# TUD-UCB-Boda/boda-1

Hardware: AMD Instinct MI355X
Metric: per-op GFLOPS and % fp32 roofline on sgemm-ops-full + conv-ops (AlexNet/NiN/GoogLeNet) (higher is better)
Workload: dtype f32; 1 GPU; sgemm-ops-full.txt + conv-ops-1-5-20-nin-alex-gn.txt + op_sigs_full.txt (one main-kernel launch per op per step); launch=hipGraph replay of each step, ops=399, units=399, ops_cut_into_panels=0, parallelism=op-shard1 (LPT, no collective), plat=hip:MI355X:gfx950:sramecc+:xnack-

## Files before the change

boda-1_amd/csrc/bh_common.h:

```cpp
#pragma once
#include <hip/hip_runtime.h>
#include <hip/hip_ext.h>
#include <stdint.h>
#include <algorithm>
#include <dlfcn.h>
#include <map>
#include <mutex>
#include <string>
#include <vector>
#include "boda_hip.h"
#include "bh_lanes.h"

namespace bh {
struct op_scope;
}
struct bh_lane {
  hipStream_t stream = nullptr;
  void *ws = nullptr;
  size_t ws_bytes = 0;
  void *cnt = nullptr;
  uint64_t cnt_n = 0;
  bool forked = false;
};
struct bh_sched {
  int lanes = 1;
  double narrow_us = 0;
  bool capturing = false;
  bh_lane lane[bh_lanes::MAX_LANES];
  std::vector<hipEvent_t> ev;
  size_t ev_used = 0;
  bh_lanes::tracker trk;
  size_t hw_ws = 0;
  bh::op_scope *scope = nullptr;
  uint32_t used_mask = 0;
  uint32_t cur[4] = {0, 0, 0, 0};
  uint32_t stats[4] = {0, 0, 0, 0};
  std::vector<uint32_t> cur_trace, trace;
};

struct bh_ctx {
  int device = 0;
  hipStream_t stream = nullptr;
  hipDeviceProp_t prop{};
  std::vector<hipEvent_t> events;
  int events_used = 0;
  int ovr_cfg[2] = {-1, -1};
  uint32_t ovr_splits[2] = {0, 0};
  int ovr_red[2] = {0, 0};
  int ovr_wt[2] = {-1, -1};
  std::vector<hipGraphExec_t> graphs;
  void *stamps = nullptr;
  hipEvent_t t_start = nullptr;
  hipEvent_t t_stop = nullptr;
  double stamp_hz = 100e6;
  void *wpack = nullptr;
  size_t wpack_bytes = 0;
  int bck_cfg[2] = {-1, -1};
  int bck_splits[2] = {0, 0};
  void *bckw = nullptr;
  size_t bckw_bytes = 0;
  std::vector<void *> retired;
  bh_sched sched;
};

namespace bh {

int fail(int code, const std::string &msg);
int ok();

int check_launch(const char *what);

int launch(bh_ctx *ctx, const void *kernel, dim3 grid, dim3 block, void **args, bool first, bool last,
           const char *what, uint32_t shmem = 0);

struct op_scope {
  bh_ctx *c;
  bh_lanes::access acc;
  double est_us = 0;
  bool narrow = false;
  bool resolved = false;
  bool pin0 = false;
  int lane = 0;
// ... 159 lines not shown
```

boda-1_amd/csrc/bh_direct.hip:

```cpp
#include "bh_gemm_dev.h"

namespace bhk {
static int launch_dc(bh_ctx *ctx, const cfg_t &c, const bh::conv_call &cc, GemmArgs &p, const route_t &r);
namespace {

template <int KX, int WPM>
constexpr int dc_koff(int tap, int KK) {
  return tap < KK ? (tap / KX) * WPM + tap % KX : 0;
}

template <int KX, int S, int WPM>
constexpr int dc_koffp(int tap, int KK) {
  return tap < KK ? (tap / KX) * WPM + ((tap % KX) % S) * (WPM / S) + (tap % KX) / S : 0;
}
template <int KY, int KX, int S, int WPM>
struct dc_pkinds {
  static constexpr int KK = KY * KX, KK2 = (KK + 1) / 2;
  struct tab_t {
    int nk;
    int dk[32];
    int kind[KK2];
  };
  static constexpr tab_t make() {
    tab_t t{};
// ... 22 lines not shown
}

template <int KY, int KX, int S, int WPM, int RIN, int TM, int TN, int D, int V4 = 0, int PSL = 0, int PFO = 0>
__global__ __launch_bounds__(256) void dc_kernel(GemmArgs p) {
  constexpr int NW = 4;
  constexpr int NPX = NW * 32 * TN, OCT = 32 * TM;
  constexpr int KK = KY * KX, KK2 = (KK + 1) / 2;
  constexpr int WPC = 2 * KK2 * OCT / 4;
  constexpr int LWA = (WPC + NW * 64 - 1) / (NW * 64);
  constexpr int WREG = LWA * NW * 256;
  constexpr int SF = RIN * WPM;
  constexpr int PW = V4 ? 4 : 1;
  static_assert(WPM % PW == 0, "16-B strip rows");
  static_assert(!PSL || (!V4 && WPM % S == 0), "phase-split strip: dword DMA, whole phases per row");
  constexpr int WS = WPM / S;
  constexpr int LWB = (SF / PW + NW * 64 - 1) / (NW * 64);
  constexpr int SREG = LWB * NW * 64 * PW;
  constexpr int BREG = NW * 64;
  constexpr int SLOT = WREG + SREG + BREG;
  constexpr int LW = LWA + LWB + 1;
  static_assert(D >= 2 && (D - 2) * LW <= 63, "vmcnt range");
  static_assert(OCT % 4 == 0 && OCT <= BREG, "16-B weight pieces, biases of one tile");
  constexpr int PF = PFO > 0 ? PFO : (TM * TN >= 4 ? 1 : (TM * TN >= 2 ? 2 : 3));
  constexpr int IS = (KK2 + 1) / 2 > 1 ? (KK2 + 1) / 2 : 1;
  constexpr int NST = TM * TN * 4;
  constexpr int ISS = KK2 > 2 * NST ? 2 * NST : KK2;
  __shared__ __attribute__((aligned(16))) float smem[D * SLOT];

  const int tid = threadIdx.x, lane = tid & 63;
  const int wave = __builtin_amdgcn_readfirstlane(tid >> 6);
  const int kh = lane >> 5, li = lane & 31;
  KT(0);

  const uint32_t G = gridDim.x, b0 = blockIdx.x;
  const uint32_t ntile = p.total_it;
  const uint32_t my_tiles = b0 < ntile ? (ntile - b0 + G - 1) / G : 0;
  auto decode = [&](uint32_t t, uint32_t &oc0, uint32_t &img, uint32_t &p0) {
    const uint32_t rest = fdiv(t, p.ipt_m, p.ipt_s);
    oc0 = (t - rest * p.ipt) * OCT;
    img = fdiv(rest, p.tm_m, p.tm_s);
    p0 = (rest - img * p.tiles_n) * NPX;
  };

  const __amdgpu_buffer_rsrc_t rsw = make_rsrc(p.a, p.a_bytes);
  const __amdgpu_buffer_rsrc_t rsi = make_rsrc(p.b, p.b_bytes);
  const __amdgpu_buffer_rsrc_t rsbias = make_rsrc(p.bias, p.bias ? p.M * 4u : 0u);
  uint32_t wrel[LWA], wc4[LWA], srel[LWB], srow[LWB];
#pragma unroll
  for (int j = 0; j < LWA; ++j) {
    const uint32_t e = (uint32_t)((wave * LWA + j) * 64 + lane);
    const uint32_t tap = e / (OCT / 4);
    wc4[j] = tap < (uint32_t)KK ? 4 * (e % (OCT / 4)) : 0xffffu;
    wrel[j] = (tap * p.IC * p.lda + 4 * (e % (OCT / 4))) * 4u;
  }
  const uint32_t pxa = V4 ? (p.px ? 4u : 0u) : p.px;
#pragma unroll
  for (int j = 0; j < LWB; ++j) {
    const uint32_t e = (uint32_t)((wave * LWB + j) * 64 + lane) * PW;
    const uint32_t r = e / WPM, q = e - (e / WPM) * WPM;
    const uint32_t c = PSL ? (q % WS) * S + q / WS : q;
    const int x = (int)c - (int)pxa;
    srow[j] = ((r < (uint32_t)RIN) & ((uint32_t)x < p.W)) ? r : 0xffffu;
    srel[j] = (r * p.W + (uint32_t)x) * 4u;
  }

  uint32_t tvo[LW];
  auto plan_tile = [&](uint32_t i) {
// ... 233 lines not shown
#endif
}

template <int KY, int KX, int S, int WPM, int RIN, int TM, int NW, int D, int V4, int ICMAX, int DBG = 0, int PFO = 0,
          int PSL = 0>
__global__ __launch_bounds__(NW * 64) void dcr_kernel(GemmArgs p) {
  constexpr int NT = NW * 64, NPX = NW * 32, OCT = 32 * TM;
  constexpr int KK = KY * KX, KK2 = (KK + 1) / 2;
  constexpr int WPC = 2 * KK2 * OCT / 4;
  constexpr int LWA = (WPC + NT - 1) / NT;
  constexpr int WREGC = LWA * NT * 4;
  constexpr int BREG = ((OCT + 63) / 64) * 64;
  constexpr int SF = RIN * WPM;
  constexpr int PW = V4 ? 4 : 1;
  static_assert(WPM % PW == 0, "16-B strip rows");
  static_assert(!PSL || (!V4 && WPM % S == 0), "phase-split strip: dword DMA, whole phases per row");
  constexpr int WS = WPM / S;
  constexpr int LWB = (SF / PW + NT - 1) / NT;
  constexpr int SREG = LWB * NT * PW;
  static_assert(D >= 2 && (D - 2) * LWB <= 63, "vmcnt range");
  static_assert(OCT % 4 == 0 && BREG <= NT, "16-B weight pieces, one bias DMA per wave at most");
  constexpr int PF = PFO > 0 ? PFO : (TM >= 2 ? 2 : 3);
  constexpr int IS = (KK2 + 1) / 2 > 1 ? (KK2 + 1) / 2 : 1;
  constexpr int NST = TM * 4;
  constexpr int ISS = KK2 > 2 * NST ? 2 * NST : KK2;
  __shared__ __attribute__((aligned(16))) float smem[ICMAX * WREGC + BREG + D * SREG];
  float *const wres = smem, *const bres = smem + ICMAX * WREGC, *const ring = bres + BREG;

  const int tid = threadIdx.x, lane = tid & 63;
  const int wave = __builtin_amdgcn_readfirstlane(tid >> 6);
  const int kh = lane >> 5, li = lane & 31;
  KT(0);

  const uint32_t G = gridDim.x, b0 = blockIdx.x;
  const uint32_t ntile = p.total_it;
  const uint32_t my_tiles = b0 < ntile ? (ntile - b0 + G - 1) / G : 0;
  const uint32_t oc0 = (b0 - fdiv(b0, p.ipt_m, p.ipt_s) * p.ipt) * OCT;
  auto decode = [&](uint32_t t, uint32_t &img, uint32_t &p0) {
    const uint32_t rest = fdiv(t, p.ipt_m, p.ipt_s);
    img = fdiv(rest, p.tm_m, p.tm_s);
    p0 = (rest - img * p.tiles_n) * NPX;
  };
  const __amdgpu_buffer_rsrc_t rsw = make_rsrc(p.a, p.a_bytes);
  const __amdgpu_buffer_rsrc_t rsi = make_rsrc(p.b, p.b_bytes);
  const __amdgpu_buffer_rsrc_t rsbias = make_rsrc(p.bias, p.bias ? p.M * 4u : 0u);

#pragma unroll
  for (int j = 0; j < LWA; ++j) {
    const uint32_t e = (uint32_t)((j * NW + wave) * 64 + lane), tap = e / (OCT / 4), c4 = 4 * (e % (OCT / 4));
    const uint32_t off = oob_unless((tap < (uint32_t)KK) & (oc0 + c4 < p.lda), (tap * p.IC * p.lda + oc0 + c4) * 4u);
    for (uint32_t ic = 0; ic < p.IC; ++ic) dma16s(rsw, wres + ic * WREGC + (j * NW + wave) * 256, off, ic * p.lda * 4u);
  }
  if (64 * wave < BREG)
    dma4(rsbias, bres + 64 * wave, oob_unless(oc0 + 64 * wave + lane < p.M, (oc0 + 64 * wave + lane) * 4u));

  const uint32_t pxa = V4 ? (p.px ? 4u : 0u) : p.px;
  uint32_t srel[LWB], srow[LWB], tvo[LWB];
#pragma unroll
  for (int j = 0; j < LWB; ++j) {
    const uint32_t e = (uint32_t)((wave * LWB + j) * 64 + lane) * PW;
    const uint32_t r = e / WPM, q = e - r * WPM;
    const uint32_t c = PSL ? (q % WS) * S + q / WS : q;
    const int x = (int)c - (int)pxa;
    srow[j] = ((r < (uint32_t)RIN) & ((uint32_t)x < p.W)) ? r : 0xffffu;
    srel[j] = (r * p.W + (uint32_t)x) * 4u;
  }
  auto plan_tile = [&](uint32_t i) {
// ... 302 lines not shown
  const uint32_t KY = cc.KY, KX = cc.KX, sy = cc.sy, sx = cc.sx;
  if ((int)KY != c.ky || (int)KX != c.kx || (int)sy != c.stride || (int)sx != c.stride)
    return bh::fail(BH_UNSUP, std::string("conv: direct config ") + c.name + " is for another kernel / stride");
  const bool v4 = c.v4 != 0;
  if (v4 && (p.W % 4 || p.px > 4))
    return bh::fail(BH_UNSUP, std::string("conv: 16-B strip pieces need W % 4 == 0, pad <= 4 for ") + c.name);
  const uint32_t pxa = v4 ? (p.px ? 4u : 0u) : p.px;
  const uint64_t maxcol = (uint64_t)pxa + (uint64_t)(p.OW - 1) * sx + KX - 1 - p.px;
  if (pxa + p.W > (uint32_t)c.wpm || maxcol >= (uint64_t)c.wpm)
    return bh::fail(BH_UNSUP, std::string("conv: input row too wide for ") + c.name);
  const uint32_t npx = (uint32_t)c.BN, OW = p.OW, OHW = p.OHW;
  const uint32_t tiles = (OHW + npx - 1) / npx;
  for (uint32_t t = 0; t < tiles; ++t) {
    const uint32_t a = t * npx, b = std::min(OHW, a + npx) - 1;
    if ((b / OW - a / OW) * sy + KY > (uint32_t)c.strip_rows)
      return bh::fail(BH_UNSUP, std::string("conv: pixel tile spans too many input rows for ") + c.name);
  }
  const uint64_t out_bytes = (uint64_t)cc.B * p.OCOHW * 4;
  if (out_bytes >= 0x7fffff00ull) return bh::fail(BH_UNSUP, "conv: output too large for the direct kernel");
  p.c_bytes = (uint32_t)out_bytes;
  const uint32_t octiles = (p.M + c.BM - 1) / c.BM;
  const uint64_t ntile = (uint64_t)cc.B * tiles * octiles;
  if (ntile >= (1u << 31)) return bh::fail(BH_UNSUP, "conv: too many tiles");
  if (c.icmax && p.IC > (uint32_t)c.icmax)
    return bh::fail(BH_UNSUP, std::string("conv: ") + c.name + " keeps at most " + std::to_string(c.icmax) +
                                  " input channels' weights resident");
  const void *k = (const void *)c.k[A_KVEC][B_DIRECT][0];
  const int bpc = bh::occupancy(k, c.NT);
  uint32_t G = (uint32_t)std::min<uint64_t>(ntile, (uint64_t)bh::num_cus(ctx) * std::min(bpc, 4));
  if (c.icmax) G = std::max(octiles, G / octiles * octiles);
  p.total_it = (uint32_t)ntile;
  p.tiles_n = tiles;
  p.ipt = octiles;
  bh::set_fd(tiles, p.tm_m, p.tm_s);
  bh::set_fd(octiles, p.ipt_m, p.ipt_s);
  bh::set_fd(OW, p.ow_m, p.ow_s);
  bh::set_trace(ctx, p);
  void *args[] = {&p};
  return bh::launch(ctx, k, dim3(G, 1, 1), dim3(c.NT), args, r.first, true, "conv_direct");
}

}
```

boda-1_amd/csrc/bh_gemm.hip:

```cpp
#include "bh_common.h"
#include "bh_gemm_dev.h"

namespace {

using namespace bhk;


template <int BM, int BN, int BK, int TM, int TN, int WAVES_M, int WAVES_N, int ALD, int BLD, int SPL>
__global__ __launch_bounds__(WAVES_M *WAVES_N * 64) void gemm_kernel(GemmArgs p) {
  constexpr int NT = WAVES_M * WAVES_N * 64;
  constexpr int WM = TM * 32, WN = TN * 32;
  static_assert(BM == WM * WAVES_M && BN == WN * WAVES_N, "tile shape");
  static_assert(BK % 8 == 0, "BK must be a multiple of 8");
  constexpr bool IM = (BLD == B_IM2COL || BLD == B_IM1X1);
  constexpr bool AMM = (ALD == A_MVEC || ALD == A_MSCALAR);
  static_assert(!IM || (NT % BN == 0), "im2col loader needs NT % BN == 0");
  constexpr int A_LDS = AMM ? BM * (BK + APAD) : BK * BM;
  constexpr int B_LDS = BK * BN;
  constexpr int AST = BK + APAD;

  __shared__ __attribute__((aligned(16))) float smem[2 * (A_LDS + B_LDS) + (IM ? BM : 0)];
  float *const As = smem;
  float *const Bs = smem + 2 * A_LDS;
  float *const Lbias = smem + 2 * (A_LDS + B_LDS);
// ... 798 lines not shown
uint32_t resolve_splits(cfg_t const &c, choice_t const &ch, uint32_t M, uint32_t N, uint32_t K, uint32_t ncu) {
  uint32_t tiles = ((M + c.BM - 1) / c.BM) * ((N + c.BN - 1) / c.BN);
  uint32_t nkt = (K + c.BK - 1) / c.BK;
  uint32_t S = ch.splits ? ch.splits : plan_splits(tiles, K, c.BK, ncu);
  S = std::max(1u, std::min(S, nkt));
  uint32_t ks = ((nkt + S - 1) / S) * c.BK;
  return (K + ks - 1) / ks;
}

int launch_gemm(bh_ctx *ctx, int op, choice_t const &ch, int ald, int bld, GemmArgs &p, const char *what,
                bool first = true) {
  cfg_t const &c = cfgs(op)[ch.cfg];
  p.tiles_m = (p.M + c.BM - 1) / c.BM;
  p.tiles_n = (p.N + c.BN - 1) / c.BN;
  bh::set_trace(ctx, p);
  const uint64_t nblk = (uint64_t)p.tiles_m * p.tiles_n;
  if (nblk > 0x7fffffffu) return bh::fail(BH_UNSUP, std::string(what) + ": grid too large");
  const uint32_t ncu = bh::num_cus(ctx);
  bh::scratch_t sc;
  p.tbm = c.BM;
  p.tbn = c.BN;
  if (bld == B_IMTAB && !c.k[ald][bld][0]) bld = B_IM2COL;
  if (bld == B_IMTAP && !c.k[ald][bld][0]) bld = B_IMT2;
  if (bld == B_IM1X1S && !c.k[ald][bld][0]) bld = B_IM1X1;
  if (is_gv(c)) {
    kern_t k = c.k[ald][bld][0];
    if (!k) return bh::fail(BH_ERR, std::string(what) + ": gv loader not instantiated");
    const uint32_t gran = (uint32_t)c.BK;
    const uint32_t ktg = (p.K + gran - 1) / gran;
    uint32_t S = ch.splits ? ch.splits : (uint32_t)std::max<uint64_t>(1, (1024 + nblk - 1) / nblk);
    S = std::max(1u, std::min(S, ktg));
    p.ks = ((ktg + S - 1) / S) * gran;
    S = (p.K + p.ks - 1) / p.ks;
    void *args[] = {&p};
    if (S > 1) {
      if (int rc = bh::scratch(ctx, (size_t)S * nblk * c.BM * c.BN * 4, nblk, sc)) return rc;
      p.ws = sc.ws;
      p.cnt = sc.cnt;
    }
    return bh::launch(ctx, (const void *)k, dim3((uint32_t)nblk, S, 1), dim3(c.NT), args, first, true, what);
  }
  if (c.family == F_STREAMK) {
    kern_t k = c.k[ald][bld][0];
    if (!k) return bh::fail(BH_ERR, std::string(what) + ": loader combination not instantiated");
    const uint32_t ipt = (p.K + c.BK - 1) / c.BK;
    if (nblk * ipt >= (1ull << 31)) return bh::fail(BH_UNSUP, std::string(what) + ": too many K iterations");
    const uint32_t dflt_bpc = (uint32_t)std::max(1, std::min(2, 163840 / c.lds_bytes));
    const bh::sk_grid g = bh::plan_sk_grid(nblk, ipt, ncu, ch.splits, dflt_bpc, 4);
    p.ipt = ipt;
    p.ipb = g.ipb;
    p.total_it = (uint32_t)g.total;
    set_fd(ipt, p.ipt_m, p.ipt_s);
    set_fd(p.tiles_m, p.tm_m, p.tm_s);
    if (int rc = bh::scratch(ctx, (size_t)2 * g.G * c.BM * c.BN * 4, nblk, sc)) return rc;
    p.ws = sc.ws;
    p.cnt = sc.cnt;
    void *args[] = {&p};
    return bh::launch(ctx, (const void *)k, dim3((uint32_t)g.G, 1, 1), dim3(c.NT), args, first, true, what);
  }
  const uint32_t S = resolve_splits(c, ch, p.M, p.N, p.K, ncu);
  const uint32_t nkt = (p.K + c.BK - 1) / c.BK;
  p.ks = ((nkt + S - 1) / S) * c.BK;
  int red = S <= 1 ? 0 : (ch.red ? ch.red : (nblk >= 64 || S > 4 ? 1 : 2));
  if (red == 2 && (uint64_t)S * nblk * c.BM * c.BN * 4 >= 0x7fffff00ull) red = 1;
  if (bld == B_IM1X1V && !c.k[ald][bld][red]) bld = B_IM1X1;
  kern_t k = c.k[ald][bld][red];
// ... 282 lines not shown
```

boda-1_amd/csrc/bh_gemm_dev.h:

```cpp
#pragma once
#include "bh_common.h"
#include "bh_skgrid.h"

namespace bhk {

typedef float f32x16 __attribute__((ext_vector_type(16)));
typedef float f32x4v __attribute__((ext_vector_type(4)));
typedef float f32x2v __attribute__((ext_vector_type(2)));

enum { A_KVEC = 0, A_KSCALAR = 1, A_MVEC = 2, A_MSCALAR = 3 };
enum { B_KVEC = 0, B_KSCALAR = 1, B_IM2COL = 2, B_IM1X1 = 3, B_IM1X1V = 4, B_IMT2 = 5, B_FC = 6, B_IMTAB = 7,
       B_IMTAP = 8, B_IM1X1S = 9, B_DIRECT = 10, NBLD = 11 };
constexpr int TAB_MAX = 512;

constexpr uint32_t OOB = 0x80000000u;
constexpr int APAD = 4;

struct GemmArgs {
  const float *a, *b;
  float *c;
  const float *bias;
  float *ws;
  uint32_t *cnt;
  uint32_t M, N, K;
  uint32_t lda, ldb, ldc;
  uint32_t tbm, tbn;
  uint32_t ks;
  uint32_t a_bytes, b_bytes;
  uint32_t c_bytes;
  uint32_t tiles_m, tiles_n;
  int relu;
  int cvec;
  int wt;
  const float *res;
  uint32_t H, W, KX, KYX, sy, sx, py, px, OW, OHW, HW, ICHW, OCOHW;
  uint32_t kyx_m, kyx_s, kx_m, kx_s, ohw_m, ohw_s, ow_m, ow_s;
  uint32_t IC, ic_m, ic_s;
  uint32_t ipt, ipb, total_it, ipt_m, ipt_s, tm_m, tm_s;
#ifdef BH_KTRACE
  unsigned long long *trace;
#endif
};

#ifdef BH_KTRACE
#define KT(k)                                                                                     \
  do {                                                                                            \
    if (threadIdx.x == 0)                                                                         \
      p.trace[((size_t)blockIdx.y * gridDim.x + blockIdx.x) * 8 + (k)] = wall_clock64();          \
  } while (0)
#else
#define KT(k) \
  do {        \
  } while (0)
#endif

__device__ __forceinline__ uint32_t fdiv(uint32_t n, uint32_t m, uint32_t s) {
  return (__umulhi(n, m) + n) >> s;
}

__device__ __forceinline__ __amdgpu_buffer_rsrc_t make_rsrc(const void *p, uint32_t bytes) {
  return __builtin_amdgcn_make_buffer_rsrc(const_cast<void *>(p), (short)0, (int)bytes, 0x00020000);
}
__device__ __forceinline__ uint32_t oob_unless(bool ok, uint32_t off) { return ok ? off : OOB; }
__device__ __forceinline__ f32x4v ld4(__amdgpu_buffer_rsrc_t r, uint32_t off) {
  return __builtin_bit_cast(f32x4v, __builtin_amdgcn_raw_buffer_load_b128(r, off, 0, 0));
}
__device__ __forceinline__ float ld1(__amdgpu_buffer_rsrc_t r, uint32_t off) {
  return __builtin_bit_cast(float, __builtin_amdgcn_raw_buffer_load_b32(r, off, 0, 0));
}

__device__ __forceinline__ uint32_t xcd_contig(uint32_t bid, uint32_t G) {
  const uint32_t xcd = bid & 7, q = G >> 3, r = G & 7;
  return (xcd < r ? xcd * (q + 1) : r * (q + 1) + (xcd - r) * q) + (bid >> 3);
}

__device__ __forceinline__ void map_tile(uint32_t bid, uint32_t tiles_m, uint32_t tiles_n, uint32_t &tm,
                                         uint32_t &tn) {
  uint32_t wgid = xcd_contig(bid, tiles_m * tiles_n);
  const uint32_t G = 8;
  uint32_t per_group = G * tiles_n;
  uint32_t group = wgid / per_group;
  uint32_t first_m = group * G;
  uint32_t gsm = min(tiles_m - first_m, G);
  uint32_t rem = wgid - group * per_group;
  tm = first_m + rem % gsm;
  tn = rem / gsm;
}

template <int N>
struct fvec;
template <>
struct fvec<1> { typedef float t; };
template <>
struct fvec<2> { typedef f32x2v t; };
template <>
struct fvec<4> { typedef f32x4v t; };

template <int N>
__device__ __forceinline__ float vget(const typename fvec<N>::t &v, int i) {
  if constexpr (N == 1) return v;
  else return v[i];
}

constexpr int AUX_SC1 = 16;
#ifndef BH_AUX_OUT
#define BH_AUX_OUT 0
#endif
// ... 277 lines not shown
```

boda-1_amd/csrc/bh_gv.hip:

```cpp
#include "bh_gemm_dev.h"

namespace bhk {
namespace {

typedef float f32x4t __attribute__((ext_vector_type(4)));


template <int R, int C, int NW>
struct gv_geom {
  static constexpr int NT = NW * 64, BMr = 16 * R, NC = 16 * C;
  static constexpr int TSZ = BMr * NC;
  static constexpr int NCH = TSZ / 4, CH = (NCH + NT - 1) / NT;
  static_assert(NCH % NT == 0 || NT % NCH == 0, "float4 chunks per thread");
};

template <int R, int C, int NW>
__device__ __forceinline__ void gv_bias(const GemmArgs &p, uint32_t m0, int tid, float (&bias_r)[gv_geom<R, C, NW>::CH]) {
  using G = gv_geom<R, C, NW>;
  const bool has = G::NCH % G::NT == 0 || tid < G::NCH;
#pragma unroll
  for (int j = 0; j < G::CH; ++j) {
    const uint32_t m = m0 + 4 * (uint32_t)(tid + j * G::NT) / G::NC;
    bias_r[j] = (has && p.bias && m < p.M) ? p.bias[m] : 0.0f;
  }
}

template <int R, int C, int NW, int RS, int CX = 1>
__device__ __forceinline__ void gv_finish(const GemmArgs &p, f32x4t (&acc)[R][C], float *red, uint32_t tm, uint32_t tn,
                                          int tid, int wave, int lane,
                                          const float (&bias_r)[gv_geom<R, C, NW>::CH]) {
  using G = gv_geom<R, C, NW>;
  constexpr int NT = G::NT, NC = G::NC, TSZ = G::TSZ, NCH = G::NCH, CH = G::CH;
  uint32_t *const flag = (uint32_t *)(red + NW * TSZ);
  const int i = lane & 15, g = lane >> 4;
  const uint32_t tile = blockIdx.x, split = blockIdx.y;
  {
    float *const Rw = red + wave * TSZ;
#pragma unroll
    for (int r = 0; r < R; ++r)
#pragma unroll
      for (int c = 0; c < C; ++c)
#pragma unroll
        for (int j = 0; j < 4; ++j) {
          const int row = RS == 1 ? 16 * r + 4 * g + j : RS * (4 * g + j) + r;
          Rw[row * NC + (CX > 1 ? CX * i + c : 16 * c + i)] = acc[r][c][j];
        }
  }
  __syncthreads();
  const bool has = NCH % NT == 0 || tid < NCH;
  f32x4v v[CH];
#pragma unroll
  for (int j = 0; j < CH; ++j) {
    const int ch = has ? tid + j * NT : 0;
    v[j] = *(const f32x4v *)&red[4 * ch];
#pragma unroll
    for (int w = 1; w < NW; ++w) v[j] += *(const f32x4v *)&red[w * TSZ + 4 * ch];
  }
  constexpr int IMODE = 1;
  if (gridDim.y == 1) {
    if (has) {
#pragma unroll
      for (int j = 0; j < CH; ++j) finish_store_b<IMODE, NC>(p, tm, tn, (uint32_t)(tid + j * NT), v[j], bias_r[j]);
    }
#ifdef BH_KTRACE
    asm volatile("s_waitcnt vmcnt(0)" ::: "memory");
    KT(4);
#endif
    return;
// ... 22 lines not shown
  f32x4v sum[CH];
#pragma unroll
  for (int j = 0; j < CH; ++j) sum[j] = f32x4v{0.0f, 0.0f, 0.0f, 0.0f};
  const uint32_t S = gridDim.y;
  for (uint32_t q = 0; q < S; q += 4) {
    f32x4v x[4][CH];
#pragma unroll
    for (int i2 = 0; i2 < 4; ++i2)
#pragma unroll
      for (int j = 0; j < CH; ++j)
        x[i2][j] = __builtin_bit_cast(
            f32x4v, __builtin_amdgcn_raw_buffer_load_b128(
                        rall, oob_unless(q + i2 < S, (q + i2) * tstep + (tile * TSZ + 4 * (uint32_t)(tid + j * NT)) * 4), 0,
                        AUX_SC1));
#pragma unroll
    for (int i2 = 0; i2 < 4; ++i2)
#pragma unroll
      for (int j = 0; j < CH; ++j)
        if (q + i2 < S) sum[j] += x[i2][j];
  }
#pragma unroll
  for (int j = 0; j < CH; ++j) finish_store_b<IMODE, NC>(p, tm, tn, (uint32_t)(tid + j * NT), sum[j], bias_r[j]);
}

template <int R, int C, int NW, int NG, int DB, int BLD>
__global__ __launch_bounds__(NW * 64) void gv_kernel(GemmArgs p) {
  using G = gv_geom<R, C, NW>;
  constexpr int BMr = G::BMr, NC = G::NC, KB = 16 * NG;
  __shared__ __attribute__((aligned(16))) float red[NW * G::TSZ + 4];

  const int tid = threadIdx.x, lane = tid & 63;
  const int wave = __builtin_amdgcn_readfirstlane(tid >> 6);
  KT(0);
  const uint32_t tm = blockIdx.x % p.tiles_m, tn = blockIdx.x / p.tiles_m, split = blockIdx.y;
  const uint32_t m0 = tm * BMr;
  const uint32_t kq = p.ks / NW;
  const uint32_t kw0 = split * p.ks + wave * kq;
  const uint32_t kw1 = min(p.K, kw0 + kq);
  const int i = lane & 15, g = lane >> 4;

  const __amdgpu_buffer_rsrc_t rsa = make_rsrc(p.a, p.a_bytes);
  const __amdgpu_buffer_rsrc_t rsb = make_rsrc(p.b, p.b_bytes);
  uint32_t arow[R];
#pragma unroll
  for (int r = 0; r < R; ++r) {
    const uint32_t m = m0 + 16 * r + i;
    arow[r] = oob_unless(m < p.M, m * p.lda * 4u);
  }
  uint32_t bcol[C];
  int iy0[C], ix0[C];
#pragma unroll
  for (int c = 0; c < C; ++c) {
    const uint32_t n = tn * NC + 16 * c + i;
    iy0[c] = 0;
    ix0[c] = 0;
    if constexpr (BLD == B_FC) {
      bcol[c] = oob_unless(n < p.N, n * p.K * 4u);
    } else {
      const uint32_t img = fdiv(n, p.ohw_m, p.ohw_s), pix = n - img * p.OHW;
      if constexpr (BLD == B_IM1X1) {
        bcol[c] = oob_unless(n < p.N, (img * p.ICHW + pix) * 4u);
      } else {
        const uint32_t oy = fdiv(pix, p.ow_m, p.ow_s), ox = pix - oy * p.OW;
        iy0[c] = (int)(oy * p.sy) - (int)p.py;
        ix0[c] = (int)(ox * p.sx) - (int)p.px;
        bcol[c] = (uint32_t)((int)(img * p.ICHW) + iy0[c] * (int)p.W + ix0[c]);
        if (n >= p.N) iy0[c] = -(1 << 29);
// ... 45 lines not shown
#pragma unroll
    for (int gg = 0; gg < NG; ++gg)
#pragma unroll
      for (int q = 0; q < 4; ++q)
#pragma unroll
        for (int r = 0; r < R; ++r)
#pragma unroll
          for (int c = 0; c < C; ++c)
            acc[r][c] = __builtin_amdgcn_mfma_f32_16x16x4f32(a[gg][r][q], b[gg][c][q], acc[r][c], 0, 0, 0);
  };
  uint32_t kb = kw0;
  if constexpr (DB) {
    if (kb < kw1) load_batch(kb, a0, b0);
    while (kb < kw1) {
      const uint32_t k1 = kb + KB;
      if (k1 < kw1) load_batch(k1, a1, b1);
      mma_batch(a0, b0);
      if (kb == kw0) KT(1);
      if (k1 >= kw1) break;
      const uint32_t k2 = k1 + KB;
      if (k2 < kw1) load_batch(k2, a0, b0);
      mma_batch(a1, b1);
      kb = k2;
    }
  } else {
    for (; kb < kw1; kb += KB) {
      load_batch(kb, a0, b0);
      mma_batch(a0, b0);
      if (kb == kw0) KT(1);
    }
  }

  KT(2);
  gv_finish<R, C, NW, 1>(p, acc, red, tm, tn, tid, wave, lane, bias_r);
}

template <int R>
__device__ __forceinline__ typename fvec<R>::t ldv(__amdgpu_buffer_rsrc_t r, uint32_t voff, uint32_t soff) {
  if constexpr (R == 4)
    return __builtin_bit_cast(f32x4v, __builtin_amdgcn_raw_buffer_load_b128(r, voff, soff, 0));
  else if constexpr (R == 2)
    return __builtin_bit_cast(f32x2v, __builtin_amdgcn_raw_buffer_load_b64(r, voff, soff, 0));
  else
    return __builtin_bit_cast(float, __builtin_amdgcn_raw_buffer_load_b32(r, voff, soff, 0));
}

template <int R, int C, int NW, int NG, int DB, int BLD, int PD = 0, int CX = 1>
__global__ __launch_bounds__(NW * 64) void gvp_kernel(GemmArgs p) {
  static_assert(BLD == B_IMTAP || BLD == B_IM1X1S || BLD == B_IM1X1 || BLD == B_FC,
                "gvp loaders: one-tap im2col, 1x1 or ipconv");
  constexpr bool AO = BLD == B_IM1X1 || BLD == B_FC;
  static_assert(CX == 1 || (CX == C && (CX == 2 || CX == 4) && BLD != B_IMTAP), "column interleave: 1x1, CX == C");
  using G = gv_geom<R, C, NW>;
  constexpr int BMr = G::BMr, NC = G::NC, KB = 16 * NG;
  typedef typename fvec<R>::t av_t;
  __shared__ __attribute__((aligned(16))) float red[NW * G::TSZ + 4];

  const int tid = threadIdx.x, lane = tid & 63;
  const int wave = __builtin_amdgcn_readfirstlane(tid >> 6);
  KT(0);
  const uint32_t tm = blockIdx.x % p.tiles_m, tn = blockIdx.x / p.tiles_m, split = blockIdx.y;
  const uint32_t m0 = tm * BMr;
  const uint32_t kq = p.ks / NW;
  const uint32_t kw0 = split * p.ks + wave * kq;
  const uint32_t kw1 = min(p.K, kw0 + kq);
  const int i = lane & 15, g = lane >> 4;
  const __amdgpu_buffer_rsrc_t rsa = make_rsrc(p.a, p.a_bytes);
  const __amdgpu_buffer_rsrc_t rsb = make_rsrc(p.b, p.b_bytes);
  const uint32_t lda4 = p.lda * 4u, hw4 = p.HW * 4u;
  const uint32_t arow = oob_unless(m0 + R * i < p.lda, (m0 + R * i) * 4u + g * lda4);
  uint32_t arow_o[AO ? R : 1];
#pragma unroll
  for (int r = 0; r < (AO ? R : 1); ++r) {
    const uint32_t m = m0 + 16 * r + i;
    arow_o[r] = oob_unless(m < p.M, (m * p.lda + 4 * g) * 4u);
  }
  uint32_t bcol[C];
  int iy0[C], ix0[C];
#pragma unroll
  for (int c = 0; c < C; ++c) {
    const uint32_t n = CX > 1 ? tn * NC + CX * i : tn * NC + 16 * c + i;
    const uint32_t img = fdiv(n, p.ohw_m, p.ohw_s), pix = n - img * p.OHW;
    iy0[c] = 0;
    ix0[c] = 0;
    if constexpr (BLD == B_FC) {
      bcol[c] = oob_unless(n < p.N, (n * p.ICHW + 4 * g) * 4u);
    } else if constexpr (BLD == B_IM1X1S || AO) {
      bcol[c] = oob_unless(n < p.N, (img * p.ICHW + pix + (AO ? 4 * g : g) * p.HW) * 4u);
    } else {
      const uint32_t oy = fdiv(pix, p.ow_m, p.ow_s), ox = pix - oy * p.OW;
      iy0[c] = (int)(oy * p.sy) - (int)p.py;
      ix0[c] = (int)(ox * p.sx) - (int)p.px;
      bcol[c] = (uint32_t)((int)(img * p.ICHW + g * p.HW) + iy0[c] * (int)p.W + ix0[c]);
      if (n >= p.N) iy0[c] = -(1 << 29);
// ... 105 lines not shown
  auto load_batch = [&](uint32_t kb, av_t(&a)[NG][4], float(&b)[NG][4][C]) {
#pragma unroll
    for (int gg = 0; gg < NG; ++gg) load_grp(kb + 16 * gg, a[gg], b[gg]);
  };
  auto mma_batch = [&](const av_t(&a)[NG][4], const float(&b)[NG][4][C]) {
#pragma unroll
    for (int gg = 0; gg < NG; ++gg) mma_grp(a[gg], b[gg]);
  };
  uint32_t kb = kw0;
  if constexpr (DB) {
    if (kb < kw1) load_batch(kb, a0, b0);
    while (kb < kw1) {
      const uint32_t k1 = kb + KB;
      if (k1 < kw1) load_batch(k1, a1, b1);
      mma_batch(a0, b0);
      if (kb == kw0) KT(1);
      if (k1 >= kw1) break;
      const uint32_t k2 = k1 + KB;
      if (k2 < kw1) load_batch(k2, a0, b0);
      mma_batch(a1, b1);
      kb = k2;
    }
  } else {
    for (; kb < kw1; kb += KB) {
      load_batch(kb, a0, b0);
      mma_batch(a0, b0);
      if (kb == kw0) KT(1);
    }
  }

  }

  KT(2);
  gv_finish<R, C, NW, AO ? 1 : R, CX>(p, acc, red, tm, tn, tid, wave, lane, bias_r);
}

template <int R, int C, int NW, int NG, int DB>
cfg_t gv_cfg(const char *name) {
  cfg_t c{name, 16 * R, 16 * C, 16 * NW, NW * 64, {}, 0};
  c.family = F_GV;
  c.k[A_MVEC][B_FC][0] = gv_kernel<R, C, NW, NG, DB, B_FC>;
  c.k[A_MVEC][B_IM1X1][0] = gv_kernel<R, C, NW, NG, DB, B_IM1X1>;
  c.k[A_MVEC][B_IM2COL][0] = gv_kernel<R, C, NW, NG, DB, B_IM2COL>;
  return c;
}

template <int R, int U, int NB>
__global__ __launch_bounds__(256) void fcv_kernel(GemmArgs p) {
  const int lane = threadIdx.x & 63;
  const int wave = __builtin_amdgcn_readfirstlane(threadIdx.x >> 6);
  const uint32_t m0 = (blockIdx.x * 4u + (uint32_t)wave) * R;
  const __amdgpu_buffer_rsrc_t rsa = make_rsrc(p.a, p.a_bytes);
  const __amdgpu_buffer_rsrc_t rsb = make_rsrc(p.b, p.b_bytes);
  const uint32_t K = p.K;
  uint32_t wrow[R], xrow[NB];
#pragma unroll
  for (int r = 0; r < R; ++r) wrow[r] = m0 + r < p.M ? (m0 + r) * K * 4u + 16u * lane : OOB;
#pragma unroll
  for (int b = 0; b < NB; ++b) xrow[b] = (uint32_t)b < p.N ? (uint32_t)b * p.ICHW * 4u + 16u * lane : OOB;
  float acc[R][NB];
#pragma unroll
  for (int r = 0; r < R; ++r)
#pragma unroll
    for (int b = 0; b < NB; ++b) acc[r][b] = 0.0f;
  for (uint32_t kc = 0; kc < K; kc += 256u * U) {
    f32x4v w[U][R], x[U][NB];
#pragma unroll
// ... 150 lines not shown
```

boda-1_amd/csrc/bh_runtime.hip:

```cpp
#include "bh_common.h"
#include <cstdio>
#include <cstring>

namespace {
thread_local std::string g_last_error;

__global__ void stamp_kernel(unsigned long long *t, int slot) {
  if (threadIdx.x == 0) t[slot] = wall_clock64();
}
__global__ void spin_kernel(unsigned long long ticks) {
  const unsigned long long t0 = wall_clock64();
  while (wall_clock64() - t0 < ticks) __builtin_amdgcn_s_sleep(8);
}
constexpr int STAMP_SLOTS = 1 << 18;
}

namespace bh {
int fail(int code, const std::string &msg) {
  g_last_error = msg;
  return code;
}
int ok() { return BH_OK; }
int check_launch(const char *what) {
  hipError_t e = hipGetLastError();
// ... 218 lines not shown
}

int bh_init(int device, bh_ctx **out) {
  if (!out) return bh::fail(BH_ERR, "null ctx out-pointer");
  *out = nullptr;
  int n = 0;
  if (hipGetDeviceCount(&n) != hipSuccess || n == 0)
    return bh::fail(BH_ERR, "no HIP device available (libboda_hip has no CPU fallback)");
  if (device < 0 || device >= n) return bh::fail(BH_ERR, "device index out of range");
  bh_ctx *c = new bh_ctx();
  c->device = device;
  hipError_t e = hipSetDevice(device);
  if (e == hipSuccess) e = hipGetDeviceProperties(&c->prop, device);
  if (e == hipSuccess && std::strncmp(c->prop.gcnArchName, "gfx950", 6) != 0) {
    std::string arch = c->prop.gcnArchName;
    delete c;
    return bh::fail(BH_ERR, "device is " + arch + "; libboda_hip is built for gfx950 (MI355X) only");
  }
  if (e == hipSuccess) e = hipMalloc(&c->stamps, STAMP_SLOTS * sizeof(unsigned long long));
  if (e == hipSuccess) {
    int khz = 0;
    e = hipDeviceGetAttribute(&khz, hipDeviceAttributeWallClockRate, device);
    c->stamp_hz = khz > 0 ? khz * 1000.0 : 100e6;
  }
  bh_sched &sc = c->sched;
  sc.lanes = bh::DEFAULT_LANES;
  sc.narrow_us = bh::DEFAULT_NARROW_US;
  if (const char *v = getenv("BH_CAPTURE_LANES")) sc.lanes = atoi(v);
  if (const char *v = getenv("BH_CAPTURE_NARROW_US")) sc.narrow_us = atof(v);
  double fork_us = bh::DEFAULT_FORK_US;
  if (const char *v = getenv("BH_CAPTURE_FORK_US")) fork_us = atof(v);
  if (const char *v = getenv("GPU_MAX_HW_QUEUES"))
    if (atoi(v) < 4) sc.lanes = 1;
  sc.lanes = std::max(1, std::min(sc.lanes, (int)bh_lanes::MAX_LANES));
  for (int k = 0; k < sc.lanes && e == hipSuccess; ++k)
    e = hipStreamCreateWithFlags(&sc.lane[k].stream, hipStreamNonBlocking);
  c->stream = sc.lane[0].stream;
  sc.trk.reset(sc.lanes);
  sc.trk.set_fork_us(fork_us);
  if (e != hipSuccess) {
    for (bh_lane &l : sc.lane)
      if (l.stream) (void)hipStreamDestroy(l.stream);
    if (c->stamps) (void)hipFree(c->stamps);
    delete c;
    return bh::fail(BH_ERR, std::string("bh_init: ") + hipGetErrorString(e));
  }
  *out = c;
  return BH_OK;
}

int bh_destroy(bh_ctx *c) {
  BH_ENTER(c);
  (void)hipSetDevice(c->device);
  (void)hipStreamSynchronize(c->stream);
  for (hipEvent_t ev : c->events) (void)hipEventDestroy(ev);
  for (hipGraphExec_t g : c->graphs)
    if (g) (void)hipGraphExecDestroy(g);
  bh::jit_release_all(c);
  for (void *r : c->retired) (void)hipFree(r);
  if (c->wpack) (void)hipFree(c->wpack);
  if (c->bckw) (void)hipFree(c->bckw);
  if (c->stamps) (void)hipFree(c->stamps);
  for (bh_lane &l : c->sched.lane) {
    if (l.stream) (void)hipStreamSynchronize(l.stream);
    if (l.ws) (void)hipFree(l.ws);
    if (l.cnt) (void)hipFree(l.cnt);
// ... 499 lines not shown
```

Measured before the change: 142,000 GFLOP/s.

## Add XCD-aware block-to-tile remapping for gemm, gv and direct conv kernels

Introduces a shared XCD mapping header that remaps hardware block IDs, which the hardware distributes round-robin across the 8 XCDs, so that each XCD gets a contiguous range of tiles in pixel-major or OC-major order. A host-side rule picks the order from operand sizes, split count and the per-XCD L2 capacity; by default (rule mode) it applies only to large-operand, unsplit cases and to direct conv with large inputs. The aim is better L2 reuse of shared A/B panels within each XCD. It adds index arithmetic per block and may hurt load balance or reuse when the heuristic picks badly.

After: 142,000 GFLOP/s. Within noise of the previous version (-0.0%).

```diff
diff --git a/boda-1_amd/csrc/bh_common.h b/boda-1_amd/csrc/bh_common.h
--- a/boda-1_amd/csrc/bh_common.h
+++ b/boda-1_amd/csrc/bh_common.h
@@ -48,6 +48,7 @@
   uint32_t ovr_splits[2] = {0, 0};
   int ovr_red[2] = {0, 0};
   int ovr_wt[2] = {-1, -1};
+  int xcd_order = 1;
   std::vector<hipGraphExec_t> graphs;
   void *stamps = nullptr;
   hipEvent_t t_start = nullptr;
diff --git a/boda-1_amd/csrc/bh_direct.hip b/boda-1_amd/csrc/bh_direct.hip
--- a/boda-1_amd/csrc/bh_direct.hip
+++ b/boda-1_amd/csrc/bh_direct.hip
@@ -78,7 +78,7 @@
   const int kh = lane >> 5, li = lane & 31;
   KT(0);
 
-  const uint32_t G = gridDim.x, b0 = blockIdx.x;
+  const uint32_t G = gridDim.x, b0 = p.xg.order == bh::XCD_HW ? blockIdx.x : xcd_contig(blockIdx.x, G);
   const uint32_t ntile = p.total_it;
   const uint32_t my_tiles = b0 < ntile ? (ntile - b0 + G - 1) / G : 0;
   auto decode = [&](uint32_t t, uint32_t &oc0, uint32_t &img, uint32_t &p0) {
@@ -378,7 +378,7 @@
   const int kh = lane >> 5, li = lane & 31;
   KT(0);
 
-  const uint32_t G = gridDim.x, b0 = blockIdx.x;
+  const uint32_t G = gridDim.x, b0 = p.xg.order == bh::XCD_HW ? blockIdx.x : xcd_contig(blockIdx.x, G);
   const uint32_t ntile = p.total_it;
   const uint32_t my_tiles = b0 < ntile ? (ntile - b0 + G - 1) / G : 0;
   const uint32_t oc0 = (b0 - fdiv(b0, p.ipt_m, p.ipt_s) * p.ipt) * OCT;
@@ -747,6 +747,8 @@
   p.total_it = (uint32_t)ntile;
   p.tiles_n = tiles;
   p.ipt = octiles;
+  p.xg.order = ctx->xcd_order == bh::XCD_MODE_ALL ? (uint32_t)bh::XCD_PIXEL
+               : ctx->xcd_order == bh::XCD_MODE_RULE ? bh::xcd_rule_direct(p.b_bytes) : (uint32_t)bh::XCD_HW;
   bh::set_fd(tiles, p.tm_m, p.tm_s);
   bh::set_fd(octiles, p.ipt_m, p.ipt_s);
   bh::set_fd(OW, p.ow_m, p.ow_s);
diff --git a/boda-1_amd/csrc/bh_gemm.hip b/boda-1_amd/csrc/bh_gemm.hip
--- a/boda-1_amd/csrc/bh_gemm.hip
+++ b/boda-1_amd/csrc/bh_gemm.hip
@@ -854,6 +854,12 @@
     S = std::max(1u, std::min(S, ktg));
     p.ks = ((ktg + S - 1) / S) * gran;
     S = (p.K + p.ks - 1) / p.ks;
+    uint32_t order = bh::XCD_HW;
+    if (nblk * S < (1ull << 31)) {
+      if (ctx->xcd_order == bh::XCD_MODE_RULE) order = bh::xcd_rule_order(p.a_bytes, p.b_bytes, p.tiles_m, p.tiles_n, S, c.BN);
+      if (ctx->xcd_order == bh::XCD_MODE_ALL) order = bh::xcd_pick_order(p.a_bytes, p.b_bytes, p.tiles_m, p.tiles_n, S);
+    }
+    p.xg = bh::xcd_make_grid(p.tiles_m, p.tiles_n, S, order);
     void *args[] = {&p};
     if (S > 1) {
       if (int rc = bh::scratch(ctx, (size_t)S * nblk * c.BM * c.BN * 4, nblk, sc)) return rc;
diff --git a/boda-1_amd/csrc/bh_gemm_dev.h b/boda-1_amd/csrc/bh_gemm_dev.h
--- a/boda-1_amd/csrc/bh_gemm_dev.h
+++ b/boda-1_amd/csrc/bh_gemm_dev.h
@@ -1,6 +1,8 @@
 #pragma once
 #include "bh_common.h"
 #include "bh_skgrid.h"
+#define BH_XCDMAP_FN __host__ __device__ __forceinline__
+#include "bh_xcdmap.h"
 
 namespace bhk {
 
@@ -37,6 +39,7 @@
   uint32_t kyx_m, kyx_s, kx_m, kx_s, ohw_m, ohw_s, ow_m, ow_s;
   uint32_t IC, ic_m, ic_s;
   uint32_t ipt, ipb, total_it, ipt_m, ipt_s, tm_m, tm_s;
+  bh::xcd_grid xg;
 #ifdef BH_KTRACE
   unsigned long long *trace;
 #endif
@@ -69,10 +72,7 @@
   return __builtin_bit_cast(float, __builtin_amdgcn_raw_buffer_load_b32(r, off, 0, 0));
 }
 
-__device__ __forceinline__ uint32_t xcd_contig(uint32_t bid, uint32_t G) {
-  const uint32_t xcd = bid & 7, q = G >> 3, r = G & 7;
-  return (xcd < r ? xcd * (q + 1) : r * (q + 1) + (xcd - r) * q) + (bid >> 3);
-}
+using bh::xcd_contig;
 
 __device__ __forceinline__ void map_tile(uint32_t bid, uint32_t tiles_m, uint32_t tiles_n, uint32_t &tm,
                                          uint32_t &tn) {
diff --git a/boda-1_amd/csrc/bh_gv.hip b/boda-1_amd/csrc/bh_gv.hip
--- a/boda-1_amd/csrc/bh_gv.hip
+++ b/boda-1_amd/csrc/bh_gv.hip
@@ -14,6 +14,14 @@
   static_assert(NCH % NT == 0 || NT % NCH == 0, "float4 chunks per thread");
 };
 
+__device__ __forceinline__ void gv_tile(const GemmArgs &p, uint32_t &tm, uint32_t &tn, uint32_t &split) {
+  const bh::xcd_tile t = p.xg.order == bh::XCD_HW ? bh::xcd_decode(blockIdx.x, blockIdx.y, p.xg)
+                                                  : bh::xcd_map(blockIdx.y * gridDim.x + blockIdx.x, p.xg);
+  tm = t.tm;
+  tn = t.tn;
+  split = t.split;
+}
+
 template <int R, int C, int NW>
 __device__ __forceinline__ void gv_bias(const GemmArgs &p, uint32_t m0, int tid, float (&bias_r)[gv_geom<R, C, NW>::CH]) {
   using G = gv_geom<R, C, NW>;
@@ -27,13 +35,13 @@
 
 template <int R, int C, int NW, int RS, int CX = 1>
 __device__ __forceinline__ void gv_finish(const GemmArgs &p, f32x4t (&acc)[R][C], float *red, uint32_t tm, uint32_t tn,
-                                          int tid, int wave, int lane,
+                                          uint32_t split, int tid, int wave, int lane,
                                           const float (&bias_r)[gv_geom<R, C, NW>::CH]) {
   using G = gv_geom<R, C, NW>;
   constexpr int NT = G::NT, NC = G::NC, TSZ = G::TSZ, NCH = G::NCH, CH = G::CH;
   uint32_t *const flag = (uint32_t *)(red + NW * TSZ);
   const int i = lane & 15, g = lane >> 4;
-  const uint32_t tile = blockIdx.x, split = blockIdx.y;
+  const uint32_t tile = tn * p.tiles_m + tm;
   {
     float *const Rw = red + wave * TSZ;
 #pragma unroll
@@ -122,7 +130,8 @@
   const int tid = threadIdx.x, lane = tid & 63;
   const int wave = __builtin_amdgcn_readfirstlane(tid >> 6);
   KT(0);
-  const uint32_t tm = blockIdx.x % p.tiles_m, tn = blockIdx.x / p.tiles_m, split = blockIdx.y;
+  uint32_t tm, tn, split;
+  gv_tile(p, tm, tn, split);
   const uint32_t m0 = tm * BMr;
   const uint32_t kq = p.ks / NW;
   const uint32_t kw0 = split * p.ks + wave * kq;
@@ -234,7 +243,7 @@
   }
 
   KT(2);
-  gv_finish<R, C, NW, 1>(p, acc, red, tm, tn, tid, wave, lane, bias_r);
+  gv_finish<R, C, NW, 1>(p, acc, red, tm, tn, split, tid, wave, lane, bias_r);
 }
 
 template <int R>
@@ -261,7 +270,8 @@
   const int tid = threadIdx.x, lane = tid & 63;
   const int wave = __builtin_amdgcn_readfirstlane(tid >> 6);
   KT(0);
-  const uint32_t tm = blockIdx.x % p.tiles_m, tn = blockIdx.x / p.tiles_m, split = blockIdx.y;
+  uint32_t tm, tn, split;
+  gv_tile(p, tm, tn, split);
   const uint32_t m0 = tm * BMr;
   const uint32_t kq = p.ks / NW;
   const uint32_t kw0 = split * p.ks + wave * kq;
@@ -433,7 +443,7 @@
   }
 
   KT(2);
-  gv_finish<R, C, NW, AO ? 1 : R, CX>(p, acc, red, tm, tn, tid, wave, lane, bias_r);
+  gv_finish<R, C, NW, AO ? 1 : R, CX>(p, acc, red, tm, tn, split, tid, wave, lane, bias_r);
 }
 
 template <int R, int C, int NW, int NG, int DB>
diff --git a/boda-1_amd/csrc/bh_runtime.hip b/boda-1_amd/csrc/bh_runtime.hip
--- a/boda-1_amd/csrc/bh_runtime.hip
+++ b/boda-1_amd/csrc/bh_runtime.hip
@@ -274,6 +274,7 @@
   if (const char *v = getenv("BH_CAPTURE_FORK_US")) fork_us = atof(v);
   if (const char *v = getenv("GPU_MAX_HW_QUEUES"))
     if (atoi(v) < 4) sc.lanes = 1;
+  if (const char *v = getenv("BH_XCD_ORDER")) c->xcd_order = std::max(0, std::min(atoi(v), 2));
   sc.lanes = std::max(1, std::min(sc.lanes, (int)bh_lanes::MAX_LANES));
   for (int k = 0; k < sc.lanes && e == hipSuccess; ++k)
     e = hipStreamCreateWithFlags(&sc.lane[k].stream, hipStreamNonBlocking);
diff --git a/boda-1_amd/csrc/bh_xcdmap.h b/boda-1_amd/csrc/bh_xcdmap.h
--- /dev/null
+++ b/boda-1_amd/csrc/bh_xcdmap.h
@@ -0,0 +1,80 @@
+#pragma once
+#include <stdint.h>
+
+#ifndef BH_XCDMAP_FN
+#define BH_XCDMAP_FN inline
+#endif
+
+namespace bh {
+
+constexpr uint32_t NUM_XCD = 8;
+
+enum { XCD_HW = 0, XCD_PIXEL = 1, XCD_OC = 2 };
+
+struct xcd_tile {
+  uint32_t tm, tn, split;
+};
+
+struct xcd_div {
+  uint32_t d, m, s;
+};
+inline xcd_div xcd_make_div(uint32_t d) {
+  xcd_div v{d ? d : 1, 0, 0};
+  while ((1ull << v.s) < v.d) ++v.s;
+  v.m = (uint32_t)(((1ull << 32) * ((1ull << v.s) - v.d)) / v.d + 1);
+  return v;
+}
+BH_XCDMAP_FN uint32_t xcd_quot(uint32_t n, const xcd_div &v) {
+  return ((uint32_t)(((uint64_t)n * v.m) >> 32) + n) >> v.s;
+}
+
+struct xcd_grid {
+  uint32_t tiles_m, tiles_n, splits, order;
+  xcd_div fast, nblk;
+};
+inline xcd_grid xcd_make_grid(uint32_t tiles_m, uint32_t tiles_n, uint32_t splits, uint32_t order) {
+  return {tiles_m, tiles_n, splits, order, xcd_make_div(order == XCD_OC ? tiles_n : tiles_m),
+          xcd_make_div(tiles_m * tiles_n)};
+}
+
+BH_XCDMAP_FN uint32_t xcd_contig(uint32_t bid, uint32_t G) {
+  const uint32_t xcd = bid & 7, q = G >> 3, r = G & 7;
+  return (xcd < r ? xcd * (q + 1) : r * (q + 1) + (xcd - r) * q) + (bid >> 3);
+}
+
+BH_XCDMAP_FN xcd_tile xcd_decode(uint32_t tile, uint32_t split, const xcd_grid &g) {
+  const uint32_t slow = xcd_quot(tile, g.fast), fast = tile - slow * g.fast.d;
+  if (g.order == XCD_OC) return {slow, fast, split};
+  return {fast, slow, split};
+}
+
+BH_XCDMAP_FN xcd_tile xcd_map(uint32_t id, const xcd_grid &g) {
+  const uint32_t l = g.order == XCD_HW ? id : xcd_contig(id, g.nblk.d * g.splits);
+  const uint32_t split = g.splits > 1 ? xcd_quot(l, g.nblk) : 0;
+  return xcd_decode(l - split * g.nblk.d, split, g);
+}
+
+inline uint32_t xcd_pick_order(uint64_t a_bytes, uint64_t b_bytes, uint32_t tiles_m, uint32_t tiles_n, uint32_t splits) {
+  const uint32_t xs = splits >= NUM_XCD ? 1 : (NUM_XCD + splits - 1) / (splits ? splits : 1);
+  const uint64_t xn = tiles_n < xs ? tiles_n : xs, xm = tiles_m < xs ? tiles_m : xs;
+  const uint64_t pixel = a_bytes * xn + b_bytes, oc = a_bytes + b_bytes * xm;
+  return tiles_m > 1 && oc < pixel ? XCD_OC : XCD_PIXEL;
+}
+
+constexpr uint64_t XCD_L2_BYTES = 4ull << 20;
+constexpr uint32_t XCD_LINE_BYTES = 128;
+
+inline uint32_t xcd_rule_order(uint64_t a_bytes, uint64_t b_bytes, uint32_t tiles_m, uint32_t tiles_n, uint32_t splits,
+                               uint32_t tile_n) {
+  const bool common = tiles_m > 1 || tile_n * 4 < XCD_LINE_BYTES;
+  return splits == 1 && b_bytes > XCD_L2_BYTES && common &&
+                 xcd_pick_order(a_bytes, b_bytes, tiles_m, tiles_n, splits) == XCD_PIXEL
+             ? XCD_PIXEL
+             : XCD_HW;
+}
+constexpr uint64_t XCD_DIRECT_BYTES = 2ull << 20;
+inline uint32_t xcd_rule_direct(uint64_t in_bytes) { return in_bytes >= XCD_DIRECT_BYTES ? XCD_PIXEL : XCD_HW; }
+
+enum { XCD_MODE_HW = 0, XCD_MODE_RULE = 1, XCD_MODE_ALL = 2 };
+
+}
```
